# REGRAGUIahmed/DGViT-Depth-Goal-Guided-Vision-Transformer-

Hardware: AMD Instinct MI355X
Metric: depth frames/sec through DGViT fwd+bwd, batch 512x84x84 (higher is better)
Workload: dtype f32

## Files before the change

### dgvit-depth-goal-guided-vision-transformer-_amd/csrc/gemm.hip

```cpp
#include <algorithm>

#include "common.h"
#include "gemm_tile.h"

namespace {

__device__ __forceinline__ void stamp(const GemmParams& p, int slot, int tid) {
#ifdef DGVIT_DIAG
  if (p.stamps && tid == 0 && (int)blockIdx.x < p.stamp_capacity) {
    long long* s = p.stamps + (long long)blockIdx.x * 16;
    s[slot] = __builtin_readcyclecounter();
    if (slot == 0) {
      s[4] = wall_clock64();
      s[5] = (long long)__builtin_amdgcn_s_getreg((31 << 11) | 4) | ((long long)__builtin_amdgcn_s_getreg((31 << 11) | 20) << 32);
    }
    if (slot == 3) s[6] = wall_clock64();
  }
#endif
}
#ifdef DGVIT_DIAG
#define DIAG_BIT(p, b) ((p).diag & (b))
#define DIAG_STAMPS(p) ((p).stamps != nullptr)
#else
#define DIAG_BIT(p, b) 0
#define DIAG_STAMPS(p) false
#endif

__device__ __forceinline__ long long unpatch_off(const GemmParams& p, int m, int k) {
  const int b = m / p.g_P, pi = m - b * p.g_P, py = pi / p.g_gw, px = pi - py * p.g_gw;
  const int i = k / p.g_pw, j = k - i * p.g_pw;
  return (long long)b * p.g_hw + (long long)(py * p.g_ph + i) * p.g_wi + px * p.g_pw + j;
}

template <class T, int LAYOUT, int VEC, int EPI, bool GATHER = false>
__global__ void __launch_bounds__(T::NT, T::MINB) gemm_f32_kernel(const GemmParams p) {
  constexpr int BM = T::BM, BN = T::BN, BK = T::BK, NT = T::NT;
  constexpr bool AKC = LAYOUT != GEMM_TN;
  constexpr bool BKC = LAYOUT == GEMM_NT;
  constexpr bool TWO_OUT = EPI == EPI_GELU2 || EPI == EPI_GELU2D;
  constexpr bool ACT_GRAD = EPI == EPI_DGELU || EPI == EPI_DMUL;
  constexpr bool NT_STORES = TWO_OUT || ACT_GRAD;
  constexpr int WM = BM / T::WVM, WN = BN / T::WVN, TM = WM / 32, TN = WN / 32;
  static_assert(WM % 32 == 0 && WN % 32 == 0 && BM <= NT, "bad wave layout");
  constexpr int A_TILE = AKC ? BM * (BK + 4) : BK * (BM + 4);
  constexpr int B_TILE = BKC ? BN * (BK + 4) : BK * (BN + 4);
  constexpr int STAGE = A_TILE + B_TILE;
  using FA = Fetch<BM, BK, AKC, VEC, NT, GATHER>;
  using FB = Fetch<BN, BK, BKC, VEC, NT>;

  extern __shared__ __attribute__((aligned(16))) float smem[];

  const int tid = threadIdx.x, lane = tid & 63, wave = tid >> 6;
  const int li = lane & 31, h = lane >> 5;
  const int wm = wave / T::WVN, wn = wave % T::WVN;

  const int tiles_n = (p.N + BN - 1) / BN, tiles_m = (p.M + BM - 1) / BM;
  int tile, zs = 0, nz = 1;
  int zslice = blockIdx.z;
  if (EPI == EPI_SPLITK && p.zsplit > 1) {
    const int ntile = tiles_m * tiles_n, w = xcd_remap(blockIdx.x, ntile * p.zsplit);
    zslice = w / ntile;
    tile = w - zslice * ntile;
  } else if (EPI != EPI_SPLITK && p.nsplit > 1 && (int)blockIdx.x >= p.split_from) {
    const int r = (int)blockIdx.x - p.split_from;
    tile = p.split_from + r / p.nsplit;
    zs = r % p.nsplit;
    nz = p.nsplit;
  } else {
    tile = xcd_remap(blockIdx.x, EPI != EPI_SPLITK && p.nsplit > 1 ? p.split_from : tiles_m * tiles_n);
  }
  const int m0 = (tile / tiles_n) * BM, n0 = (tile % tiles_n) * BN;
  const int kbeg = nz > 1 ? zs * p.kchunk_split : zslice * p.kchunk;
  const int kend = min(p.K, kbeg + (nz > 1 ? p.kchunk_split : p.kchunk));
  const int nk = kend > kbeg ? (kend - kbeg + BK - 1) / BK : 0;

  f32x16 acc[TM][TN];
#pragma unroll
  for (int i = 0; i < TM; ++i)
#pragma unroll
    for (int j = 0; j < TN; ++j)
#pragma unroll
      for (int r = 0; r < 16; ++r) acc[i][j][r] = 0.f;

  float bsum = 0.f;
  const bool do_colsum = EPI == EPI_SPLITK && p.colsum && n0 == 0 && tid < BM;

  float4 ra[FA::NV], rb[FB::NV];
  const int klim = kend - kbeg;
  stamp(p, 0, tid);

  constexpr bool ELEMWISE = BM == 64 && BN == 64 && BK == 32;
  constexpr bool LN_OK = EPI == EPI_STORE && BN == 64 && VEC == 4 && !GATHER && LAYOUT != GEMM_TN;
  const bool evec = !ELEMWISE || p.evec;
  constexpr int CS = BN + 4;
  constexpr int NCHUNK = (BM * CS <= 2 * STAGE) ? 1 : T::WVM;
  constexpr int CROWS = BM / NCHUNK;
  static_assert(CROWS * CS <= 2 * STAGE && (NCHUNK == 1 || CROWS == WM), "epilogue C image does not fit the staging LDS");
  constexpr int C4 = BN / 4, RPP = NT / C4;
  const int cc = (tid % C4) * 4, rr0 = tid / C4;
  const int n = n0 + cc;
  constexpr bool DIRECT_OK = LAYOUT != GEMM_TN && VEC == 4 && !GATHER && EPI != EPI_SPLITK && EPI != EPI_UNPATCH && (BKC || TN <= 2);
  const bool direct = DIRECT_OK && nz == 1 && evec && p.c_rgrp == 0 && p.res_mod == 0 && (!TWO_OUT || p.ldc2 == p.ldc) && !DIAG_BIT(p, 8) &&
                      !(LN_OK && p.ln_y);
  int dcol[TN];
  float dbias[TN];
#pragma unroll
  for (int j = 0; j < TN; ++j) {
    dcol[j] = wn * WN + (BKC ? j * 32 + li : li * TN + j);
    dbias[j] = 0.f;
  }
  float bias4[4] = {0.f, 0.f, 0.f, 0.f};
  if ((EPI == EPI_STORE || TWO_OUT || EPI == EPI_RELU || EPI == EPI_GELU) && p.bias) {
    if (direct) {
#pragma unroll
      for (int j = 0; j < TN; ++j) dbias[j] = p.bias[min(n0 + dcol[j], p.N - 1)];
    } else {
#pragma unroll
      for (int e = 0; e < 4; ++e)
        if (n + e < p.N) bias4[e] = p.bias[n + e];
    }
  }

  auto load_frags = [&](float (&fa)[TM][4], float (&fb)[TN][4], const float* la, const float* lb, int g) {
    if constexpr (AKC) {
#pragma unroll
      for (int i = 0; i < TM; ++i) frag<BM, BK, true>(fa[i], la, wm * WM + i * 32 + li, g, h);
    } else {
      frag_mc<BM, TM>(fa, la, wm * WM, li, g, h);
    }
    if constexpr (BKC) {
#pragma unroll
      for (int j = 0; j < TN; ++j) frag<BN, BK, true>(fb[j], lb, wn * WN + j * 32 + li, g, h);
    } else {
      frag_mc<BN, TN>(fb, lb, wn * WN, li, g, h);
    }
  };
  auto do_mfma = [&](const float (&fa)[TM][4], const float (&fb)[TN][4]) {
#pragma unroll
    for (int s4 = 0; s4 < 4; ++s4)
#pragma unroll
      for (int i = 0; i < TM; ++i)
#pragma unroll
        for (int j = 0; j < TN; ++j)
          acc[i][j] = __builtin_amdgcn_mfma_f32_32x32x2f32(fa[i][s4], fb[j][s4], acc[i][j], 0, 0, 0);
  };
  auto mma_group = [&](const float* la, const float* lb, int g) {
    float fa[TM][4], fb[TN][4];
    load_frags(fa, fb, la, lb, g);
    do_mfma(fa, fb);
  };

  if (VEC == 4) {
    typename FA::Plan pa;
    typename FB::Plan pb;
    if constexpr (GATHER) FA::plan_gather(pa, p, m0, kbeg, tid);
    else FA::plan(pa, p.A, p.lda, m0, p.M, kbeg, p.K, tid);
    FB::plan(pb, p.B, p.ldb, n0, p.N, kbeg, p.K, tid);
    {
      float4 ra0[FA::NV], rb0[FB::NV];
      FA::run4(ra0, pa, 0, klim);
      FB::run4(rb0, pb, 0, klim);
      FA::run4(ra, pa, 1, klim);
      FB::run4(rb, pb, 1, klim);
      FA::stash(ra0, smem, tid);
      FB::stash(rb0, smem + A_TILE, tid);
    }
    __syncthreads();
    stamp(p, 1, tid);
    if (DIAG_BIT(p, 1)) __builtin_amdgcn_s_setprio(2);
    for (int kt = 0; kt < nk; ++kt) {
      const float* la = smem + (kt & 1) * STAGE;
      const float* lb = la + A_TILE;
      float* wa = smem + ((kt + 1) & 1) * STAGE;
      float fa[2][TM][4], fb[2][TN][4];
      load_frags(fa[0], fb[0], la, lb, 0);
      FA::stash(ra, wa, tid);
      FB::stash(rb, wa + A_TILE, tid);
      FA::run4(ra, pa, kt + 2, klim);
      FB::run4(rb, pb, kt + 2, klim);
#pragma unroll
      for (int g = 0; g < BK / 8; ++g) {
        if (g + 1 < BK / 8) load_frags(fa[(g + 1) & 1], fb[(g + 1) & 1], la, lb, g + 1);
        do_mfma(fa[g & 1], fb[g & 1]);
      }
      sched_pattern<4 * TM * TN, FA::NV + FB::NV, (AKC ? TM : (TM == 1 ? 2 : 4)) + (BKC ? TN : (TN == 1 ? 2 : 4)), BK / 8>();
      if (EPI == EPI_SPLITK && do_colsum) {
#pragma unroll 8
        for (int kk = 0; kk < BK; ++kk) bsum += la[kk * (BM + 4) + tid];
      }
      __syncthreads();
    }
    if (DIAG_BIT(p, 1)) __builtin_amdgcn_s_setprio(0);
  } else {
    FA::run(ra, p.A, p.lda, m0, p.M, kbeg, kend, tid);
    FB::run(rb, p.B, p.ldb, n0, p.N, kbeg, kend, tid);
    FA::stash(ra, smem, tid);
    FB::stash(rb, smem + A_TILE, tid);
    __syncthreads();
    for (int kt = 0; kt < nk; ++kt) {
      const float* la = smem + (kt & 1) * STAGE;
      const float* lb = la + A_TILE;
      const bool more = kt + 1 < nk;
      if (more) {
        FA::run(ra, p.A, p.lda, m0, p.M, kbeg + (kt + 1) * BK, kend, tid);
        FB::run(rb, p.B, p.ldb, n0, p.N, kbeg + (kt + 1) * BK, kend, tid);
      }
#pragma unroll
      for (int g = 0; g < BK / 8; ++g) mma_group(la, lb, g);
      if (EPI == EPI_SPLITK && do_colsum) {
#pragma unroll 8
        for (int kk = 0; kk < BK; ++kk) bsum += la[kk * (BM + 4) + tid];
      }
      if (more) {
        float* wa = smem + ((kt + 1) & 1) * STAGE;
        FA::stash(ra, wa, tid);
        FB::stash(rb, wa + A_TILE, tid);
      }
      __syncthreads();
    }
  }

  stamp(p, 2, tid);
  if (DIAG_BIT(p, 2)) {
    float sacc = 0.f;
#pragma unroll
    for (int i = 0; i < TM; ++i)
#pragma unroll
      for (int j = 0; j < TN; ++j)
#pragma unroll
        for (int r = 0; r < 16; ++r) sacc += acc[i][j][r];
    if (sacc == 1.2345678e33f) p.C[0] = sacc;
    return;
  }
  if constexpr (DIRECT_OK) {
    if (direct) {
      constexpr int CW = BKC ? 1 : TN;
      auto tile_rsrc = [&](const float* base, int ld) {
        long long bytes = ((long long)(p.M - 1 - m0) * ld + (p.N - n0)) * 4;
        if (bytes > 0x7FFFFFFFll) bytes = 0x7FFFFFFFll;
        return __builtin_amdgcn_make_buffer_rsrc(const_cast<float*>(base + (long long)m0 * ld + n0), 0, (int)bytes, 0x00020000);
      };
      auto eoff = [&](int i, int j, int r, int ld) -> unsigned {
        const unsigned rowpart = (unsigned)((wm * WM + i * 32 + (r & 3) + 8 * (r >> 2)) * ld * 4);
        return n0 + dcol[j] < p.N ? rowpart + (unsigned)((4 * h * ld + dcol[j]) * 4) : DGVIT_OOB;
      };
      constexpr bool HAS_SIDE = EPI == EPI_STORE || ACT_GRAD || EPI == EPI_DRELU;
      const bool use_side = HAS_SIDE && (EPI == EPI_STORE ? p.res != nullptr : true);
      if (HAS_SIDE && use_side) {
        const float* sb = EPI == EPI_STORE ? p.res : p.aux;
        const int sld = EPI == EPI_STORE ? p.ldr : p.ldaux;
        const __amdgpu_buffer_rsrc_t sr = tile_rsrc(sb, sld);
        float side[TM][16][TN];
#pragma unroll
        for (int i = 0; i < TM; ++i)
#pragma unroll
          for (int r = 0; r < 16; ++r) {
            if constexpr (CW == 2) {
              typedef float f32x2v __attribute__((ext_vector_type(2)));
              const f32x2v v2 = __builtin_bit_cast(f32x2v, __builtin_amdgcn_raw_buffer_load_b64(sr, eoff(i, 0, r, sld), 0, 0));
              side[i][r][0] = v2[0];
              side[i][r][1] = v2[1];
            } else {
#pragma unroll
              for (int j = 0; j < TN; ++j)
                side[i][r][j] = __builtin_bit_cast(float, __builtin_amdgcn_raw_buffer_load_b32(sr, eoff(i, j, r, sld), 0, 0));
            }
          }
#pragma unroll
        for (int i = 0; i < TM; ++i)
#pragma unroll
          for (int j = 0; j < TN; ++j)
#pragma unroll
            for (int r = 0; r < 16; ++r) {
              const float sv = side[i][r][j];
              if (EPI == EPI_STORE) acc[i][j][r] += sv;
              else if (EPI == EPI_DGELU) acc[i][j][r] *= gelu_erf_grad(sv);
              else if (EPI == EPI_DMUL) acc[i][j][r] *= sv;
              else acc[i][j][r] = sv > 0.f ? acc[i][j][r] : 0.f;
            }
      }
      auto st32 = [&](unsigned v, __amdgpu_buffer_rsrc_t rs, unsigned off) {
        if (NT_STORES || DIAG_BIT(p, 16)) __builtin_amdgcn_raw_buffer_store_b32(v, rs, off, 0, 2);
        else __builtin_amdgcn_raw_buffer_store_b32(v, rs, off, 0, 0);
      };
      auto st64 = [&](u32x2 v, __amdgpu_buffer_rsrc_t rs, unsigned off) {
        if (NT_STORES || DIAG_BIT(p, 16)) __builtin_amdgcn_raw_buffer_store_b64(v, rs, off, 0, 2);
        else __builtin_amdgcn_raw_buffer_store_b64(v, rs, off, 0, 0);
      };
      const __amdgpu_buffer_rsrc_t cr = tile_rsrc(p.C, p.ldc);
      __amdgpu_buffer_rsrc_t c2r = cr;
      if (TWO_OUT) c2r = tile_rsrc(p.C2, p.ldc2);
#pragma unroll
      for (int i = 0; i < TM; ++i)
#pragma unroll
        for (int r = 0; r < 16; ++r) {
          float v[TN];
#pragma unroll
          for (int j = 0; j < TN; ++j) {
            v[j] = acc[i][j][r];
            if (EPI == EPI_STORE || TWO_OUT) v[j] += dbias[j];
            else if (EPI == EPI_RELU) v[j] = fmaxf(v[j] + dbias[j], 0.f);
            else if (EPI == EPI_GELU) v[j] = gelu_erf(v[j] + dbias[j]);
          }
          if constexpr (CW == 1) {
#pragma unroll
            for (int j = 0; j < TN; ++j) {
              if constexpr (EPI == EPI_GELU2D) {
                float gl, gd;
                gelu_erf_both(v[j], gl, gd);
                st32(__builtin_bit_cast(unsigned, gd), cr, eoff(i, j, r, p.ldc));
                st32(__builtin_bit_cast(unsigned, gl), c2r, eoff(i, j, r, p.ldc));
              } else {
                st32(__builtin_bit_cast(unsigned, v[j]), cr, eoff(i, j, r, p.ldc));
                if (EPI == EPI_GELU2)
                  st32(__builtin_bit_cast(unsigned, gelu_erf(v[j])), c2r, eoff(i, j, r, p.ldc));
              }
            }
          } else {
            u32x2 w;
// ... 79 lines not shown
#pragma unroll
      for (int e = 0; e < 4; ++e) v[e] += bias4[e];
    } else if (TWO_OUT) {
#pragma unroll
      for (int e = 0; e < 4; ++e) {
        v[e] += bias4[e];
        if constexpr (EPI == EPI_GELU2D) gelu_erf_both(v[e], w2[e], v[e]);
        else w2[e] = gelu_erf(v[e]);
      }
    } else if (EPI == EPI_RELU) {
#pragma unroll
      for (int e = 0; e < 4; ++e) v[e] = fmaxf(v[e] + bias4[e], 0.f);
    } else if (EPI == EPI_GELU) {
#pragma unroll
      for (int e = 0; e < 4; ++e) v[e] = gelu_erf(v[e] + bias4[e]);
    } else if (ACT_GRAD || EPI == EPI_DRELU) {
      const float* ap = p.aux + (long long)m * p.ldaux + n;
      float a4[4] = {0.f, 0.f, 0.f, 0.f};
      if (evec) {
        const float4 q = *reinterpret_cast<const float4*>(ap);
        a4[0] = q.x; a4[1] = q.y; a4[2] = q.z; a4[3] = q.w;
      } else {
#pragma unroll
        for (int e = 0; e < 4; ++e)
          if (n + e < p.N) a4[e] = ap[e];
      }
#pragma unroll
      for (int e = 0; e < 4; ++e) v[e] = EPI == EPI_DGELU ? v[e] * gelu_erf_grad(a4[e]) : (EPI == EPI_DMUL ? v[e] * a4[e] : (a4[e] > 0.f ? v[e] : 0.f));
    }
    if (evec) {
      *reinterpret_cast<float4*>(cptr) = make_float4(v[0], v[1], v[2], v[3]);
      if (TWO_OUT) *reinterpret_cast<float4*>(p.C2 + (long long)m * p.ldc2 + n) = make_float4(w2[0], w2[1], w2[2], w2[3]);
      if (LN_OK && p.ln_y) ln_piece(m, v);
    } else {
#pragma unroll
      for (int e = 0; e < 4; ++e)
        if (n + e < p.N) {
          cptr[e] = v[e];
          if (TWO_OUT) p.C2[(long long)m * p.ldc2 + n + e] = w2[e];
        }
    }
  };
  float* slab = nullptr;
  if (EPI != EPI_SPLITK && nz > 1) slab = p.slabs + ((long long)(tile - p.split_from) * nz + zs) * (BM * BN);
  constexpr int NP = CROWS / RPP;
  static_assert(CROWS % RPP == 0, "epilogue row pieces");
  constexpr bool HAS_SIDE = EPI == EPI_STORE || ACT_GRAD || EPI == EPI_DRELU;
  constexpr bool SIDE_ALL = NCHUNK == 1 && NP <= 4;
  const bool fast = evec && !slab;
  const bool nvalid = n < p.N;
  const int nc = nvalid ? n : 0;
  const bool use_side = HAS_SIDE && (EPI == EPI_STORE ? p.res != nullptr : true);
  float4 side[HAS_SIDE ? (SIDE_ALL ? NCHUNK * NP : NP) : 1];
#pragma unroll
  for (auto& sv : side) sv = make_float4(0.f, 0.f, 0.f, 0.f);
  auto load_side = [&](int ch, float4* dst) {
#pragma unroll
    for (int it = 0; it < NP; ++it) {
      const int m = min(m0 + ch * CROWS + rr0 + it * RPP, p.M - 1);
      const float* sp;
      if (EPI == EPI_STORE) {
        const long long rrow = p.res_mod > 0 ? (long long)(m % p.res_mod) + 1 : (long long)m;
        sp = p.res + rrow * p.ldr + nc;
      } else {
        sp = p.aux + (long long)m * p.ldaux + nc;
      }
      dst[it] = *reinterpret_cast<const float4*>(sp);
    }
  };
  if (HAS_SIDE && SIDE_ALL && fast && use_side) {
#pragma unroll
    for (int ch = 0; ch < NCHUNK; ++ch) load_side(ch, side + ch * NP);
  }
#pragma unroll
  for (int ch = 0; ch < NCHUNK; ++ch) {
    if (NCHUNK == 1 || wm == ch) {
      const int rbase = NCHUNK == 1 ? wm * WM : 0;
#pragma unroll
      for (int i = 0; i < TM; ++i)
#pragma unroll
        for (int r = 0; r < 16; ++r) {
          const int rt = (r & 3) + 8 * (r >> 2) + 4 * h;
          float* crow = smem + (rbase + (AKC ? i * 32 + rt : rt * TM + i)) * CS + wn * WN;
          if constexpr (BKC || TN == 1) {
#pragma unroll
            for (int j = 0; j < TN; ++j) crow[j * 32 + li] = acc[i][j][r];
          } else {
            typedef float cvec_t __attribute__((ext_vector_type(TN)));
            cvec_t v;
#pragma unroll
            for (int j = 0; j < TN; ++j) v[j] = acc[i][j][r];
            *reinterpret_cast<cvec_t*>(crow + li * TN) = v;
          }
        }
    }
    __syncthreads();
    stamp(p, 8 + 2 * ch, tid);
    if (slab) {
      const __amdgpu_buffer_rsrc_t srs = __builtin_amdgcn_make_buffer_rsrc(slab, 0, BM * BN * 4, 0x00020000);
      for (int rr = rr0; rr < CROWS; rr += RPP) {
        const float4 t = *reinterpret_cast<const float4*>(smem + rr * CS + cc);
        __builtin_amdgcn_raw_buffer_store_b128(__builtin_bit_cast(u32x4, t), srs, (unsigned)(((ch * CROWS + rr) * BN + cc) * 4), 0, 16);
      }
    } else if (fast) {
      if (HAS_SIDE && !SIDE_ALL && use_side) load_side(ch, side);
      float4* sd = side + (HAS_SIDE && SIDE_ALL ? ch * NP : 0);
      if (EPI == EPI_DGELU) {
#pragma unroll
        for (int it = 0; it < NP; ++it)
          sd[it] = make_float4(gelu_erf_grad(sd[it].x), gelu_erf_grad(sd[it].y), gelu_erf_grad(sd[it].z), gelu_erf_grad(sd[it].w));
      }
      constexpr bool T_FIRST = NCHUNK == 1;
      float4 t[T_FIRST ? NP : 1];
      if constexpr (T_FIRST) {
#pragma unroll
        for (int it = 0; it < NP; ++it) t[it] = *reinterpret_cast<const float4*>(smem + (rr0 + it * RPP) * CS + cc);
      }
#pragma unroll
      for (int it = 0; it < NP; ++it) {
        const int m = m0 + ch * CROWS + rr0 + it * RPP;
        if constexpr (!T_FIRST) t[0] = *reinterpret_cast<const float4*>(smem + (rr0 + it * RPP) * CS + cc);
        const float4 tv = t[T_FIRST ? it : 0];
        float v[4] = {tv.x, tv.y, tv.z, tv.w}, w2[4];
        if (EPI == EPI_STORE) {
          if (use_side) { v[0] += sd[it].x; v[1] += sd[it].y; v[2] += sd[it].z; v[3] += sd[it].w; }
#pragma unroll
          for (int e = 0; e < 4; ++e) v[e] += bias4[e];
        } else if (TWO_OUT) {
#pragma unroll
          for (int e = 0; e < 4; ++e) {
            v[e] += bias4[e];
            if constexpr (EPI == EPI_GELU2D) gelu_erf_both(v[e], w2[e], v[e]);
            else w2[e] = gelu_erf(v[e]);
          }
        } else if (EPI == EPI_RELU) {
#pragma unroll
          for (int e = 0; e < 4; ++e) v[e] = fmaxf(v[e] + bias4[e], 0.f);
        } else if (EPI == EPI_GELU) {
#pragma unroll
          for (int e = 0; e < 4; ++e) v[e] = gelu_erf(v[e] + bias4[e]);
        } else if (ACT_GRAD || EPI == EPI_DRELU) {
          const float a4[4] = {sd[it].x, sd[it].y, sd[it].z, sd[it].w};
#pragma unroll
          for (int e = 0; e < 4; ++e) v[e] = ACT_GRAD ? v[e] * a4[e] : (a4[e] > 0.f ? v[e] : 0.f);
        }
        if (EPI == EPI_UNPATCH && m < p.M && nvalid) {
          *reinterpret_cast<float4*>(Cz + unpatch_off(p, m, n)) = make_float4(v[0], v[1], v[2], v[3]);
        } else if (EPI != EPI_UNPATCH && m < p.M && nvalid) {
          long long crow = m;
          if (EPI == EPI_STORE && p.c_rgrp > 0) crow = (long long)m + m / p.c_rgrp + 1;
          int ncol = n;
          if (DIAG_BIT(p, 4)) {
            crow = m - m0;
            ncol = cc;
          }
          *reinterpret_cast<float4*>(Cz + crow * p.ldc + ncol) = make_float4(v[0], v[1], v[2], v[3]);
          if (TWO_OUT) *reinterpret_cast<float4*>(p.C2 + crow * p.ldc2 + ncol) = make_float4(w2[0], w2[1], w2[2], w2[3]);
          if (LN_OK && p.ln_y) ln_piece(m, v);
        }
      }
    } else if (ELEMWISE && n < p.N) {
      for (int it = 0; it < CROWS / RPP; ++it) {
        const int rr = rr0 + it * RPP;
        const int m = m0 + ch * CROWS + rr;
        if (m < p.M) {
          const float4 t = *reinterpret_cast<const float4*>(smem + rr * CS + cc);
          float v[4] = {t.x, t.y, t.z, t.w};
// ... 252 lines not shown
```

### dgvit-depth-goal-guided-vision-transformer-_amd/csrc/gemm_tile.h

```cpp
#pragma once
#include "common.h"

namespace {

template <int BM_, int BN_, int BK_, int WVM_ = 2, int WVN_ = 2>
struct TileCfg {
  static constexpr int BM = BM_, BN = BN_, BK = BK_, WVM = WVM_, WVN = WVN_, NT = 64 * WVM_ * WVN_;
  static constexpr int LDS_BYTES = 2 * (BM_ + BN_) * (BK_ + 4) * 4;
  static constexpr int MINB = LDS_BYTES * 5 <= 160 * 1024 ? 5 : 2;
};

__device__ __forceinline__ int xcd_remap(int id, int n) {
  const int q = n >> 3, r = n & 7, xcd = id & 7, loc = id >> 3;
  return (xcd < r ? xcd * (q + 1) : r * (q + 1) + (xcd - r) * q) + loc;
}

typedef unsigned u32x4 __attribute__((ext_vector_type(4)));
typedef unsigned u32x2 __attribute__((ext_vector_type(2)));
#define DGVIT_OOB 0xFFFFFFF0u

template <int R, int BK, bool KC, int VEC, int NT, bool GATHER = false>
struct Fetch {
  static_assert(!GATHER || (KC && VEC == 4), "the patch gather is a k-contiguous float4 fetch");
  static_assert(R * BK / 4 % NT == 0, "tile must split evenly over the workgroup's threads");
  static constexpr int NV = R * BK / 4 / NT;
  static constexpr int PER_ROW = KC ? BK / 4 : R / 4;

  struct Plan {
    __amdgpu_buffer_rsrc_t rsrc;
    unsigned off[NV];
    int kc[NV];
    unsigned bad[NV];
    unsigned kstep;
    int g_wi, g_pw, g_inv, g_shift;
    int g_k0;
  };

  __device__ static __forceinline__ void plan_gather(Plan& pl, const GemmParams& p, int r0, int kbeg, int tid) {
    pl.g_k0 = kbeg;
    long long bytes = p.g_img_floats * 4;
    if (bytes > 0x7FFFFFFFll) bytes = 0x7FFFFFFFll;
    pl.rsrc = __builtin_amdgcn_make_buffer_rsrc(const_cast<float*>(p.g_img), 0, (int)bytes, 0x00020000);
    pl.kstep = 0;
    pl.g_wi = p.g_wi; pl.g_pw = p.g_pw; pl.g_inv = p.g_inv; pl.g_shift = p.g_shift ? p.g_shift : 16;
    const int xs = p.g_xs ? p.g_xs : p.g_pw;
#pragma unroll
    for (int i = 0; i < NV; ++i) {
      const int f = tid + i * NT;
      const int a = f / PER_ROW, c = (f % PER_ROW) * 4;
      const int m = r0 + a;
      const int b = m / p.g_P, pi = m - b * p.g_P, hy = pi / p.g_gw, wx = pi - hy * p.g_gw;
      pl.off[i] = ((unsigned)b * (unsigned)p.g_hw + (unsigned)(hy * p.g_ph) * (unsigned)p.g_wi + (unsigned)(wx * xs)) * 4u;
      pl.kc[i] = c;
      pl.bad[i] = m < p.M ? 0u : 0xFFFFFFFFu;
    }
  }

  __device__ static __forceinline__ void plan(Plan& pl, const float* base, int ld, int r0, int rmax, int kbeg, int ktotal,
                                              int tid) {
    long long first, last;
    if (KC) {
      first = (long long)r0 * ld + kbeg;
      last = (long long)(rmax - 1) * ld + ktotal;
    } else {
      first = (long long)kbeg * ld + r0;
      last = (long long)(ktotal - 1) * ld + rmax;
    }
    long long bytes = (last - first) * 4;
    if (bytes > 0x7FFFFFFFll) bytes = 0x7FFFFFFFll;
    if (bytes < 0) bytes = 0;
    pl.rsrc = __builtin_amdgcn_make_buffer_rsrc(const_cast<float*>(base + first), 0, (int)bytes, 0x00020000);
    pl.kstep = KC ? BK * 4u : (unsigned)BK * (unsigned)ld * 4u;
#pragma unroll
    for (int i = 0; i < NV; ++i) {
      const int f = tid + i * NT;
      const int a = f / PER_ROW, c = (f % PER_ROW) * 4;
      if (KC) {
        pl.off[i] = ((unsigned)a * (unsigned)ld + (unsigned)c) * 4u;
        pl.kc[i] = c;
        pl.bad[i] = 0u;
      } else {
        pl.off[i] = ((unsigned)a * (unsigned)ld + (unsigned)c) * 4u;
        pl.kc[i] = a;
        pl.bad[i] = r0 + c < rmax ? 0u : 0xFFFFFFFFu;
      }
    }
  }

  __device__ static __forceinline__ void run4(float4 (&reg)[NV], const Plan& pl, int t, int klim) {
#pragma unroll
    for (int i = 0; i < NV; ++i) {
      unsigned at;
      if constexpr (GATHER) {
        const unsigned k = (unsigned)(pl.g_k0 + t * BK + pl.kc[i]), p1 = (k * (unsigned)pl.g_inv) >> pl.g_shift, p2 = k - p1 * (unsigned)pl.g_pw;
        at = (pl.off[i] + (p1 * (unsigned)pl.g_wi + p2) * 4u) | pl.bad[i];
      } else {
        at = (pl.off[i] + (unsigned)t * pl.kstep) | pl.bad[i];
      }
      const unsigned o = t * BK + pl.kc[i] < klim ? at : DGVIT_OOB;
      reg[i] = __builtin_bit_cast(float4, __builtin_amdgcn_raw_buffer_load_b128(pl.rsrc, o, 0, 0));
    }
  }

  __device__ static __forceinline__ void run(float4 (&reg)[NV], const float* __restrict__ base, int ld, int r0,
                                             int rmax, int k0, int kend, int tid) {
#pragma unroll
    for (int i = 0; i < NV; ++i) {
      const int f = tid + i * NT;
      const int a = f / PER_ROW, c = (f % PER_ROW) * 4;
      float4 v = make_float4(0.f, 0.f, 0.f, 0.f);
      if (KC) {
        const int row = r0 + a, k = k0 + c;
        if (row < rmax) {
          const float* src = base + (long long)row * ld + k;
          if (k + 0 < kend) v.x = src[0];
          if (k + 1 < kend) v.y = src[1];
          if (k + 2 < kend) v.z = src[2];
          if (k + 3 < kend) v.w = src[3];
        }
      } else {
        const int k = k0 + a, col = r0 + c;
        if (k < kend) {
          const float* src = base + (long long)k * ld + col;
          if (col + 0 < rmax) v.x = src[0];
          if (col + 1 < rmax) v.y = src[1];
          if (col + 2 < rmax) v.z = src[2];
          if (col + 3 < rmax) v.w = src[3];
        }
      }
      reg[i] = v;
    }
  }

  __device__ static __forceinline__ void stash(const float4 (&reg)[NV], float* lds, int tid) {
    constexpr int STRIDE = KC ? BK + 4 : R + 4;
#pragma unroll
    for (int i = 0; i < NV; ++i) {
      const int f = tid + i * NT;
      const int a = f / PER_ROW, c = (f % PER_ROW) * 4;
      *reinterpret_cast<float4*>(lds + a * STRIDE + c) = reg[i];
    }
  }
};

template <int R, int BK, bool KC>
__device__ __forceinline__ void frag(float (&out)[4], const float* lds, int row, int g, int h) {
  if (KC) {
    const float4 v = *reinterpret_cast<const float4*>(lds + row * (BK + 4) + 8 * g + 4 * h);
    out[0] = v.x; out[1] = v.y; out[2] = v.z; out[3] = v.w;
  } else {
    const float* p = lds + (8 * g + 4 * h) * (R + 4) + row;
#pragma unroll
    for (int s = 0; s < 4; ++s) out[s] = p[s * (R + 4)];
  }
}

template <int R, int NTILE>
__device__ __forceinline__ void frag_mc(float (&out)[NTILE][4], const float* lds, int base, int li, int g, int h) {
  typedef float vec_t __attribute__((ext_vector_type(NTILE == 1 ? 1 : NTILE == 2 ? 2 : 4)));
  static_assert(NTILE == 1 || NTILE == 2 || NTILE == 4, "frag_mc: tiles per wave");
  const float* p = lds + (8 * g + 4 * h) * (R + 4) + base + NTILE * li;
#pragma unroll
  for (int s = 0; s < 4; ++s) {
    if constexpr (NTILE == 1) {
      out[0][s] = p[s * (R + 4)];
    } else {
      typedef __attribute__((address_space(3))) const volatile vec_t lds_vec_t;
      const vec_t v = *(lds_vec_t*)(p + s * (R + 4));
#pragma unroll
      for (int t = 0; t < NTILE; ++t) out[t][s] = v[t];
    }
  }
}

#define SGB(mask, n) __builtin_amdgcn_sched_group_barrier(mask, n, 0)
constexpr int cdiv_c(int a, int b) { return (a + b - 1) / b; }
template <int m, int H, int NI, int MASK>
__device__ __forceinline__ void spread() {
  if constexpr (m < H) {
    SGB(0x8, 1);
    constexpr int c = cdiv_c((m + 1) * NI, H) - cdiv_c(m * NI, H);
    if constexpr (c > 0) SGB(MASK, c);
    spread<m + 1, H, NI, MASK>();
  }
}
template <int MF, int NW, int RPG, int NG>
__device__ __forceinline__ void sched_pattern() {
  static_assert(MF >= 2 && MF % 2 == 0, "sched_pattern: MFMAs per k-group");
  SGB(0x100, RPG);
  spread<0, MF / 2, NW, 0x200>();
  if constexpr (NG > 1) SGB(0x100, RPG);
  spread<0, MF / 2, NW, 0x20>();
  if constexpr (NG > 1) { if constexpr (NG > 2) SGB(0x100, RPG); SGB(0x8, MF); }
  if constexpr (NG > 2) { if constexpr (NG > 3) SGB(0x100, RPG); SGB(0x8, MF); }
  if constexpr (NG > 3) { if constexpr (NG > 4) SGB(0x100, RPG); SGB(0x8, MF); }
// ... 9 lines not shown
```

### dgvit-depth-goal-guided-vision-transformer-_amd/csrc/last_block.hip

```cpp
#include <math.h>

#include <algorithm>

#include "kernels.h"

#define DGVIT_LOG2E 1.4426950408889634f

namespace {

constexpr int GP_WAVES = 4;
constexpr int GP_J = 4;
constexpr int HP_FRAMES = 16;
constexpr int HP_CHUNK = 256;
constexpr int WG_ROWS = 8;

__device__ __forceinline__ float fma4(const float4 a, const float4 b, float acc) {
  acc = fmaf(a.x, b.x, acc);
  acc = fmaf(a.y, b.y, acc);
  acc = fmaf(a.z, b.z, acc);
  return fmaf(a.w, b.w, acc);
}
__device__ __forceinline__ void axpy4(float a, const float4 x, float4& acc) {
  acc.x = fmaf(a, x.x, acc.x);
  acc.y = fmaf(a, x.y, acc.y);
  acc.z = fmaf(a, x.z, acc.z);
  acc.w = fmaf(a, x.w, acc.w);
}

__device__ __forceinline__ void fma4v(const float4 a, const float4 b, float4& acc) {
  acc.x = fmaf(a.x, b.x, acc.x);
  acc.y = fmaf(a.y, b.y, acc.y);
  acc.z = fmaf(a.z, b.z, acc.z);
  acc.w = fmaf(a.w, b.w, acc.w);
}
__device__ __forceinline__ float4 add4(const float4 a, const float4 b) { return make_float4(a.x + b.x, a.y + b.y, a.z + b.z, a.w + b.w); }
__device__ __forceinline__ float hsum4(const float4 a) { return (a.x + a.y) + (a.z + a.w); }

template <int J>
__device__ __forceinline__ void pool_rows(const float* __restrict__ w, const float4* __restrict__ xs4, int N, int D4, int lane, float4 (&out)[J]) {
  float4 acc[4][J];
#pragma unroll
  for (int k = 0; k < 4; ++k)
#pragma unroll
    for (int j = 0; j < J; ++j) acc[k][j] = make_float4(0.f, 0.f, 0.f, 0.f);
  int t = 0;
  for (; t + 3 < N; t += 4) {
    const float4 wv = *reinterpret_cast<const float4*>(w + t);
    const float wk[4] = {wv.x, wv.y, wv.z, wv.w};
#pragma unroll
    for (int k = 0; k < 4; ++k)
#pragma unroll
      for (int j = 0; j < J; ++j) {
        const int c = lane + 64 * j;
        if (c < D4) axpy4(wk[k], xs4[(t + k) * D4 + c], acc[k][j]);
      }
  }
  for (; t < N; ++t) {
    const float wt = w[t];
#pragma unroll
    for (int j = 0; j < J; ++j) {
      const int c = lane + 64 * j;
      if (c < D4) axpy4(wt, xs4[t * D4 + c], acc[0][j]);
    }
  }
#pragma unroll
  for (int j = 0; j < J; ++j) out[j] = add4(add4(acc[0][j], acc[1][j]), add4(acc[2][j], acc[3][j]));
}

__device__ __forceinline__ void stage_frame(const float* __restrict__ xn, float4* __restrict__ xs4, int b, int N, int D) {
  const float4* src = reinterpret_cast<const float4*>(xn + (long long)b * N * D);
  const int n4 = N * (D >> 2);
  for (int i = threadIdx.x; i < n4; i += blockDim.x) xs4[i] = src[i];
}

template <int J>
__global__ void __launch_bounds__(64 * GP_WAVES) goal_pool_fwd_kernel(const float* __restrict__ xn, const float* __restrict__ u, long long fs_u,
                                                                      float* __restrict__ r, long long fs_r, float* __restrict__ p, int N,
                                                                      int D, int H, float qscale) {
  extern __shared__ float4 gp_smem[];
  float4* xs4 = gp_smem;
  const int b = blockIdx.x, D4 = D >> 2, NP = (N + 3) & ~3;
  float* sc = reinterpret_cast<float*>(gp_smem) + (long long)N * D + (threadIdx.x >> 6) * NP;
  stage_frame(xn, xs4, b, N, D);
  __syncthreads();
  const int lane = threadIdx.x & 63;
  for (int h = threadIdx.x >> 6; h < H; h += GP_WAVES) {
    const float4* uh = reinterpret_cast<const float4*>(u + (long long)b * fs_u + (long long)h * D);
    float4 uf[J];
#pragma unroll
    for (int j = 0; j < J; ++j) {
      const int c = lane + 64 * j;
      uf[j] = c < D4 ? uh[c] : make_float4(0.f, 0.f, 0.f, 0.f);
    }
    for (int t = 0; t < N; ++t) {
      float part = 0.f;
#pragma unroll
      for (int j = 0; j < J; ++j) {
        const int c = lane + 64 * j;
        if (c < D4) part = fma4(uf[j], xs4[t * D4 + c], part);
      }
      part = wave_sum(part);
      if (lane == 0) sc[t] = part * qscale;
    }
    __builtin_amdgcn_wave_barrier();
    float m = -INFINITY;
    for (int t = lane; t < N; t += 64) m = fmaxf(m, sc[t]);
    m = wave_max(m);
    float l = 0.f;
    for (int t = lane; t < N; t += 64) {
      const float e = __builtin_amdgcn_exp2f(sc[t] - m);
      sc[t] = e;
      l += e;
    }
    l = wave_sum(l);
    const float inv = 1.f / l;
    for (int t = lane; t < N; t += 64) {
      const float pt = sc[t] * inv;
      sc[t] = pt;
      if (p) p[((long long)b * H + h) * N + t] = pt;
    }
    __builtin_amdgcn_wave_barrier();
    float4 acc[J];
    pool_rows<J>(sc, xs4, N, D4, lane, acc);
    float4* rh = reinterpret_cast<float4*>(r + (long long)b * fs_r + (long long)h * D);
#pragma unroll
    for (int j = 0; j < J; ++j) {
      const int c = lane + 64 * j;
      if (c < D4) rh[c] = acc[j];
    }
  }
}

template <int J>
__global__ void __launch_bounds__(64 * GP_WAVES) goal_pool_bwd_kernel(const float* __restrict__ xn, const float* __restrict__ p,
                                                                      const float* __restrict__ u, long long fs_u, const float* __restrict__ dr,
                                                                      float* __restrict__ du, long long fs_d, float* __restrict__ dxn, int N,
                                                                      int D, int H, float scale) {
  extern __shared__ float4 gp_smem[];
  float4* xs4 = gp_smem;
  const int b = blockIdx.x, D4 = D >> 2, NP = (N + 3) & ~3;
  float* ps = reinterpret_cast<float*>(gp_smem) + (long long)N * D;
  float* das = ps + H * NP;
  stage_frame(xn, xs4, b, N, D);
  __syncthreads();
  const int lane = threadIdx.x & 63;
  for (int h = threadIdx.x >> 6; h < H; h += GP_WAVES) {
    const float4* drh = reinterpret_cast<const float4*>(dr + (long long)b * fs_d + (long long)h * D);
    float4 df[J];
#pragma unroll
    for (int j = 0; j < J; ++j) {
      const int c = lane + 64 * j;
      df[j] = c < D4 ? drh[c] : make_float4(0.f, 0.f, 0.f, 0.f);
    }
    float* dh_ = das + h * NP;
    float* ph_ = ps + h * NP;
    for (int t = 0; t < N; ++t) {
      float part = 0.f;
#pragma unroll
      for (int j = 0; j < J; ++j) {
        const int c = lane + 64 * j;
        if (c < D4) part = fma4(df[j], xs4[t * D4 + c], part);
      }
      part = wave_sum(part);
      if (lane == 0) dh_[t] = part;
    }
    __builtin_amdgcn_wave_barrier();
    float cpart = 0.f;
    for (int t = lane; t < N; t += 64) {
      const float pt = p[((long long)b * H + h) * N + t];
      ph_[t] = pt;
      cpart = fmaf(pt, dh_[t], cpart);
    }
    const float cs = wave_sum(cpart);
    for (int t = lane; t < N; t += 64) dh_[t] = scale * (ph_[t] * (dh_[t] - cs));
    __builtin_amdgcn_wave_barrier();
    float4 acc[J];
    pool_rows<J>(dh_, xs4, N, D4, lane, acc);
    float4* duh = reinterpret_cast<float4*>(du + (long long)b * fs_d + (long long)h * D);
#pragma unroll
    for (int j = 0; j < J; ++j) {
      const int c = lane + 64 * j;
      if (c < D4) duh[c] = acc[j];
    }
  }
  __syncthreads();
  const float4* dr4 = reinterpret_cast<const float4*>(dr + (long long)b * fs_d);
  const float4* u4 = reinterpret_cast<const float4*>(u + (long long)b * fs_u);
  float4* out4 = reinterpret_cast<float4*>(dxn + (long long)b * N * D);
  const int items = ((N + 3) >> 2) * D4;
  for (int it = threadIdx.x; it < items; it += blockDim.x) {
    const int t0 = (it / D4) * 4, c = it % D4;
    float4 acc[4];
#pragma unroll
    for (int k = 0; k < 4; ++k) acc[k] = make_float4(0.f, 0.f, 0.f, 0.f);
    for (int h = 0; h < H; ++h) {
      const float4 dv = dr4[h * D4 + c], uv = u4[h * D4 + c];
      const float4 pv = *reinterpret_cast<const float4*>(ps + h * NP + t0);
      const float4 av = *reinterpret_cast<const float4*>(das + h * NP + t0);
      axpy4(pv.x, dv, acc[0]); axpy4(av.x, uv, acc[0]);
      axpy4(pv.y, dv, acc[1]); axpy4(av.y, uv, acc[1]);
      axpy4(pv.z, dv, acc[2]); axpy4(av.z, uv, acc[2]);
      axpy4(pv.w, dv, acc[3]); axpy4(av.w, uv, acc[3]);
    }
#pragma unroll
    for (int k = 0; k < 4; ++k)
      if (t0 + k < N) out4[(t0 + k) * D4 + c] = acc[k];
  }
}

template <int DH>
__global__ void __launch_bounds__(256) head_proj_kernel(const float* __restrict__ in, long long ld_in, const float* __restrict__ W,
                                                        float* __restrict__ out, long long fs_out, int B, int D) {
  __shared__ float4 in_s[HP_FRAMES][DH / 4];
  const int b0 = blockIdx.x * HP_FRAMES, h = blockIdx.y;
  for (int i = threadIdx.x; i < HP_FRAMES * (DH / 4); i += 256) {
    const int f = i / (DH / 4), k4 = i % (DH / 4);
    in_s[f][k4] = b0 + f < B ? *reinterpret_cast<const float4*>(in + (long long)(b0 + f) * ld_in + h * DH + 4 * k4) : make_float4(0.f, 0.f, 0.f, 0.f);
  }
  __syncthreads();
  for (int d = threadIdx.x; d < D; d += 256) {
    float4 acc[HP_FRAMES];
#pragma unroll
    for (int f = 0; f < HP_FRAMES; ++f) acc[f] = make_float4(0.f, 0.f, 0.f, 0.f);
    const float* wp = W + (long long)h * DH * D + d;
#pragma unroll 2
    for (int k4 = 0; k4 < DH / 4; ++k4) {
      const float4 w = make_float4(wp[(long long)(4 * k4) * D], wp[(long long)(4 * k4 + 1) * D], wp[(long long)(4 * k4 + 2) * D],
                                   wp[(long long)(4 * k4 + 3) * D]);
#pragma unroll
      for (int f = 0; f < HP_FRAMES; ++f) fma4v(in_s[f][k4], w, acc[f]);
    }
#pragma unroll
    for (int f = 0; f < HP_FRAMES; ++f)
      if (b0 + f < B) out[(long long)(b0 + f) * fs_out + (long long)h * D + d] = hsum4(acc[f]);
  }
}

template <int DH>
__global__ void __launch_bounds__(256) head_proj_t_kernel(const float* __restrict__ in, long long fs_in, const float* __restrict__ W,
                                                          float* __restrict__ out, long long ld_out, int B, int D) {
  constexpr int FPT = HP_FRAMES * DH / 256;
  __shared__ float4 in_s[HP_FRAMES][HP_CHUNK / 4];
  const int b0 = blockIdx.x * HP_FRAMES, h = blockIdx.y;
  const int j = threadIdx.x % DH, f0 = (threadIdx.x / DH) * FPT;
  const float* wrow = W + ((long long)h * DH + j) * D;
  float4 acc[FPT][4];
#pragma unroll
  for (int i = 0; i < FPT; ++i)
#pragma unroll
    for (int k = 0; k < 4; ++k) acc[i][k] = make_float4(0.f, 0.f, 0.f, 0.f);
  for (int d0 = 0; d0 < D; d0 += HP_CHUNK) {
    const int dc4 = (D - d0 < HP_CHUNK ? D - d0 : HP_CHUNK) >> 2;
    __syncthreads();
    for (int i = threadIdx.x; i < HP_FRAMES * dc4; i += 256) {
      const int f = i / dc4, c = i % dc4;
      in_s[f][c] = b0 + f < B ? *reinterpret_cast<const float4*>(in + (long long)(b0 + f) * fs_in + (long long)h * D + d0 + 4 * c)
                              : make_float4(0.f, 0.f, 0.f, 0.f);
    }
    __syncthreads();
    int c = 0;
    for (; c + 3 < dc4; c += 4) {
#pragma unroll
      for (int k = 0; k < 4; ++k) {
        const float4 w = *reinterpret_cast<const float4*>(wrow + d0 + 4 * (c + k));
#pragma unroll
        for (int i = 0; i < FPT; ++i) fma4v(in_s[f0 + i][c + k], w, acc[i][k]);
      }
    }
    for (; c < dc4; ++c) {
      const float4 w = *reinterpret_cast<const float4*>(wrow + d0 + 4 * c);
#pragma unroll
      for (int i = 0; i < FPT; ++i) fma4v(in_s[f0 + i][c], w, acc[i][0]);
    }
  }
#pragma unroll
  for (int i = 0; i < FPT; ++i)
    if (b0 + f0 + i < B)
      out[(long long)(b0 + f0 + i) * ld_out + h * DH + j] = hsum4(add4(add4(acc[i][0], acc[i][1]), add4(acc[i][2], acc[i][3])));
}

template <int DH>
__global__ void __launch_bounds__(256) head_proj_wgrad_kernel(const float* __restrict__ q, long long ld_q, const float* __restrict__ du,
                                                              long long fs_du, const float* __restrict__ dout, long long ld_do,
                                                              const float* __restrict__ r, long long fs_r, float* __restrict__ dW, int B,
                                                              int D, int H, int vec) {
  __shared__ float4 red[3][WG_ROWS][64];
  constexpr int RT = DH / WG_ROWS;
  const int z = blockIdx.z, h = blockIdx.y, rt = blockIdx.x % RT, cb = blockIdx.x / RT;
  const float* A = z ? dout : q;
  const long long lda = z ? ld_do : ld_q;
  const float* X = z ? r : du;
  const long long fsx = z ? fs_r : fs_du;
  const int lane = threadIdx.x & 63, wave = threadIdx.x >> 6;
  const int c = cb * 64 + lane, D4 = D >> 2;
  const bool valid = c < D4;
  const int chunk = (B + 3) >> 2;
  const int bb = wave * chunk, be = bb + chunk < B ? bb + chunk : B;
  float4 acc[WG_ROWS];
#pragma unroll
  for (int i = 0; i < WG_ROWS; ++i) acc[i] = make_float4(0.f, 0.f, 0.f, 0.f);
  if (valid) {
    for (int b = bb; b < be; ++b) {
      const float4 x = *reinterpret_cast<const float4*>(X + (long long)b * fsx + (long long)h * D + 4 * c);
      const float* ap = A + (long long)b * lda + h * DH + rt * WG_ROWS;
      const float4 a0 = *reinterpret_cast<const float4*>(ap), a1 = *reinterpret_cast<const float4*>(ap + 4);
      axpy4(a0.x, x, acc[0]); axpy4(a0.y, x, acc[1]); axpy4(a0.z, x, acc[2]); axpy4(a0.w, x, acc[3]);
      axpy4(a1.x, x, acc[4]); axpy4(a1.y, x, acc[5]); axpy4(a1.z, x, acc[6]); axpy4(a1.w, x, acc[7]);
    }
  }
  if (wave > 0) {
#pragma unroll
    for (int i = 0; i < WG_ROWS; ++i) red[wave - 1][i][lane] = acc[i];
  }
  __syncthreads();
  if (wave == 0 && valid) {
    const long long I = (long long)H * DH;
    float* o = dW + (z * I + (long long)h * DH + rt * WG_ROWS) * D + 4 * c;
#pragma unroll
    for (int i = 0; i < WG_ROWS; ++i) {
      float4 s = acc[i];
#pragma unroll
      for (int w = 0; w < 3; ++w) {
        const float4 v = red[w][i][lane];
        s.x += v.x; s.y += v.y; s.z += v.z; s.w += v.w;
      }
      float* oi = o + (long long)i * D;
      if (vec) *reinterpret_cast<float4*>(oi) = s;
      else { oi[0] = s.x; oi[1] = s.y; oi[2] = s.z; oi[3] = s.w; }
    }
  }
}

template <int J>
int launch_pool_fwd(const float* xn, const float* u, long long fs_u, float* r, long long fs_r, float* p, int B, int N, int D, int H, float scale,
                    hipStream_t st) {
  auto kern = goal_pool_fwd_kernel<J>;
  TRY(allow_dynamic_lds<goal_pool_fwd_kernel<J>>((int)GOAL_POOL_LDS_MAX, "goal_pool_fwd"));
  const long long np = (N + 3) & ~3;
  const size_t lds = (size_t)((long long)N * D + GP_WAVES * np) * sizeof(float);
  {
    ProfileScope t(PROF_ATTN_FWD, 4.0 * B * H * (double)N * D, st);
    hipLaunchKernelGGL(kern, dim3(B), dim3(64 * GP_WAVES), lds, st, xn, u, fs_u, r, fs_r, p, N, D, H, scale * DGVIT_LOG2E);
  }
  DGVIT_CHECK_LAUNCH("goal_pool_fwd");
  return DGVIT_OK;
}

template <int J>
int launch_pool_bwd(const float* xn, const float* p, const float* u, long long fs_u, const float* dr, float* du, long long fs_d, float* dxn,
                    int B, int N, int D, int H, float scale, hipStream_t st) {
  auto kern = goal_pool_bwd_kernel<J>;
  TRY(allow_dynamic_lds<goal_pool_bwd_kernel<J>>((int)GOAL_POOL_LDS_MAX, "goal_pool_bwd"));
  const long long np = (N + 3) & ~3;
  const size_t lds = (size_t)((long long)N * D + 2ll * H * np) * sizeof(float);
  {
    ProfileScope t(PROF_ATTN_BWD, 8.0 * B * H * (double)N * D, st);
    hipLaunchKernelGGL(kern, dim3(B), dim3(64 * GP_WAVES), lds, st, xn, p, u, fs_u, dr, du, fs_d, dxn, N, D, H, scale);
  }
  DGVIT_CHECK_LAUNCH("goal_pool_bwd");
  return DGVIT_OK;
}

}

long long goal_pool_lds_bytes(int N, int D, int H) {
  const long long np = (N + 3) & ~3;
  const long long extra = std::max<long long>(GP_WAVES, 2ll * H) * np;
  return ((long long)N * D + extra) * (long long)sizeof(float);
}

bool goal_attention_supports(int N, int D, int H, int dh) {
  return N >= 1 && H >= 1 && D >= 4 && D % 4 == 0 && D <= 256 * GP_J && (dh == 32 || dh == 64) && goal_pool_lds_bytes(N, D, H) <= GOAL_POOL_LDS_MAX;
}

#define GOAL_CHECK_SHAPE(name)                                                                                                       \
  DGVIT_CHECK_ARG(B > 0 && goal_attention_supports(N, D, H, dh),                                                                    \
                  name ": unsupported shape B=%d N=%d H=%d dim_head=%d dim=%d (dim_head 32 or 64, dim a multiple of 4 up to 1024, "  \
                       "N * dim floats within %d KB of LDS)", B, N, H, dh, D, (int)(GOAL_POOL_LDS_MAX / 1024))

int head_proj(const float* in, long long ld_in, const float* W, float* out, long long fs_out, int B, int H, int dh, int D, hipStream_t st) {
  DGVIT_CHECK_ARG(in && W && out && al16(in) && ld_in % 4 == 0, "head_proj: bad arguments");
  const dim3 grid((B + HP_FRAMES - 1) / HP_FRAMES, H);
  {
    ProfileScope t(PROF_OTHER, 2.0 * B * H * (double)dh * D, st);
    if (dh == 64) hipLaunchKernelGGL(head_proj_kernel<64>, grid, dim3(256), 0, st, in, ld_in, W, out, fs_out, B, D);
    else hipLaunchKernelGGL(head_proj_kernel<32>, grid, dim3(256), 0, st, in, ld_in, W, out, fs_out, B, D);
  }
  DGVIT_CHECK_LAUNCH("head_proj");
  return DGVIT_OK;
}
// ... 69 lines not shown
```

Measured before the change: 41280.

## Pair B columns in GEMM fetch and batch loads in last-block attention kernels

Adds a paired-row permutation to the B operand fetch when TN==2 with k-contiguous B, so each lane owns adjacent output columns and the epilogue can use vector stores. In the last-block kernels it also batches independent global and LDS loads ahead of the FMAs: tokens are processed in groups of eight with a shared wave reduction, frame staging is unrolled, heads are blocked by four, and the weight-gradient loop takes eight frames per step with WG_ROWS halved to four. The intent is more memory-level parallelism and fewer serialized wave reductions, at the cost of extra registers and possible occupancy loss.

Measured after the change: 41570, median of 6. About the same (+0.7%).

```diff
diff --git a/dgvit-depth-goal-guided-vision-transformer-_amd/csrc/gemm.hip b/dgvit-depth-goal-guided-vision-transformer-_amd/csrc/gemm.hip
--- a/dgvit-depth-goal-guided-vision-transformer-_amd/csrc/gemm.hip
+++ b/dgvit-depth-goal-guided-vision-transformer-_amd/csrc/gemm.hip
@@ -46,7 +46,8 @@
   constexpr int B_TILE = BKC ? BN * (BK + 4) : BK * (BN + 4);
   constexpr int STAGE = A_TILE + B_TILE;
   using FA = Fetch<BM, BK, AKC, VEC, NT, GATHER>;
-  using FB = Fetch<BN, BK, BKC, VEC, NT>;
+  constexpr bool BPAIR = BKC && TN == 2, BTILED = BKC && !BPAIR;
+  using FB = Fetch<BN, BK, BKC, VEC, NT, false, BPAIR>;
 
   extern __shared__ __attribute__((aligned(16))) float smem[];
 
@@ -106,7 +107,7 @@
   float dbias[TN];
 #pragma unroll
   for (int j = 0; j < TN; ++j) {
-    dcol[j] = wn * WN + (BKC ? j * 32 + li : li * TN + j);
+    dcol[j] = wn * WN + (BTILED ? j * 32 + li : li * TN + j);
     dbias[j] = 0.f;
   }
   float bias4[4] = {0.f, 0.f, 0.f, 0.f};
@@ -234,7 +235,7 @@
   }
   if constexpr (DIRECT_OK) {
     if (direct) {
-      constexpr int CW = BKC ? 1 : TN;
+      constexpr int CW = BTILED ? 1 : TN;
       auto tile_rsrc = [&](const float* base, int ld) {
         long long bytes = ((long long)(p.M - 1 - m0) * ld + (p.N - n0)) * 4;
         if (bytes > 0x7FFFFFFFll) bytes = 0x7FFFFFFFll;
@@ -480,7 +481,7 @@
         for (int r = 0; r < 16; ++r) {
           const int rt = (r & 3) + 8 * (r >> 2) + 4 * h;
           float* crow = smem + (rbase + (AKC ? i * 32 + rt : rt * TM + i)) * CS + wn * WN;
-          if constexpr (BKC || TN == 1) {
+          if constexpr (BTILED || TN == 1) {
 #pragma unroll
             for (int j = 0; j < TN; ++j) crow[j * 32 + li] = acc[i][j][r];
           } else {
diff --git a/dgvit-depth-goal-guided-vision-transformer-_amd/csrc/gemm_tile.h b/dgvit-depth-goal-guided-vision-transformer-_amd/csrc/gemm_tile.h
--- a/dgvit-depth-goal-guided-vision-transformer-_amd/csrc/gemm_tile.h
+++ b/dgvit-depth-goal-guided-vision-transformer-_amd/csrc/gemm_tile.h
@@ -19,9 +19,11 @@
 typedef unsigned u32x2 __attribute__((ext_vector_type(2)));
 #define DGVIT_OOB 0xFFFFFFF0u
 
-template <int R, int BK, bool KC, int VEC, int NT, bool GATHER = false>
+template <int R, int BK, bool KC, int VEC, int NT, bool GATHER = false, bool PAIRED = false>
 struct Fetch {
   static_assert(!GATHER || (KC && VEC == 4), "the patch gather is a k-contiguous float4 fetch");
+  static_assert(!PAIRED || (KC && !GATHER && R % 64 == 0), "column pairs: a k-contiguous operand in 64-row wave blocks");
+  __device__ static __forceinline__ int src_row(int a) { return PAIRED ? (a & ~63) + 2 * (a & 31) + ((a >> 5) & 1) : a; }
   static_assert(R * BK / 4 % NT == 0, "tile must split evenly over the workgroup's threads");
   static constexpr int NV = R * BK / 4 / NT;
   static constexpr int PER_ROW = KC ? BK / 4 : R / 4;
@@ -76,7 +78,7 @@
       const int f = tid + i * NT;
       const int a = f / PER_ROW, c = (f % PER_ROW) * 4;
       if (KC) {
-        pl.off[i] = ((unsigned)a * (unsigned)ld + (unsigned)c) * 4u;
+        pl.off[i] = ((unsigned)src_row(a) * (unsigned)ld + (unsigned)c) * 4u;
         pl.kc[i] = c;
         pl.bad[i] = 0u;
       } else {
@@ -110,7 +112,7 @@
       const int a = f / PER_ROW, c = (f % PER_ROW) * 4;
       float4 v = make_float4(0.f, 0.f, 0.f, 0.f);
       if (KC) {
-        const int row = r0 + a, k = k0 + c;
+        const int row = r0 + src_row(a), k = k0 + c;
         if (row < rmax) {
           const float* src = base + (long long)row * ld + k;
           if (k + 0 < kend) v.x = src[0];
diff --git a/dgvit-depth-goal-guided-vision-transformer-_amd/csrc/last_block.hip b/dgvit-depth-goal-guided-vision-transformer-_amd/csrc/last_block.hip
--- a/dgvit-depth-goal-guided-vision-transformer-_amd/csrc/last_block.hip
+++ b/dgvit-depth-goal-guided-vision-transformer-_amd/csrc/last_block.hip
@@ -10,9 +10,13 @@
 
 constexpr int GP_WAVES = 4;
 constexpr int GP_J = 4;
+constexpr int GP_TB = 8;
+constexpr int GP_STAGE = 8;
+constexpr int GP_HB = 4;
 constexpr int HP_FRAMES = 16;
 constexpr int HP_CHUNK = 256;
-constexpr int WG_ROWS = 8;
+constexpr int WG_ROWS = 4;
+constexpr int WG_FRAMES = 8;
 
 __device__ __forceinline__ float fma4(const float4 a, const float4 b, float acc) {
   acc = fmaf(a.x, b.x, acc);
@@ -43,34 +47,81 @@
   for (int k = 0; k < 4; ++k)
 #pragma unroll
     for (int j = 0; j < J; ++j) acc[k][j] = make_float4(0.f, 0.f, 0.f, 0.f);
+  int cc[J];
+#pragma unroll
+  for (int j = 0; j < J; ++j) cc[j] = lane + 64 * j < D4 ? lane + 64 * j : 0;
   int t = 0;
   for (; t + 3 < N; t += 4) {
     const float4 wv = *reinterpret_cast<const float4*>(w + t);
     const float wk[4] = {wv.x, wv.y, wv.z, wv.w};
 #pragma unroll
-    for (int k = 0; k < 4; ++k)
-#pragma unroll
-      for (int j = 0; j < J; ++j) {
-        const int c = lane + 64 * j;
-        if (c < D4) axpy4(wk[k], xs4[(t + k) * D4 + c], acc[k][j]);
-      }
+    for (int j = 0; j < J; ++j) {
+      float4 x[4];
+#pragma unroll
+      for (int k = 0; k < 4; ++k) x[k] = xs4[(t + k) * D4 + cc[j]];
+#pragma unroll
+      for (int k = 0; k < 4; ++k) axpy4(wk[k], x[k], acc[k][j]);
+    }
   }
   for (; t < N; ++t) {
     const float wt = w[t];
 #pragma unroll
+    for (int j = 0; j < J; ++j) axpy4(wt, xs4[t * D4 + cc[j]], acc[0][j]);
+  }
+#pragma unroll
+  for (int j = 0; j < J; ++j) out[j] = add4(add4(acc[0][j], acc[1][j]), add4(acc[2][j], acc[3][j]));
+}
+
+template <int J>
+__device__ __forceinline__ void dot_rows(const float4 (&f)[J], const float4* __restrict__ xs4, int N, int D4, int lane, float mul,
+                                         float* __restrict__ out) {
+  for (int t0 = 0; t0 < N; t0 += GP_TB) {
+    float part[GP_TB];
+#pragma unroll
+    for (int k = 0; k < GP_TB; ++k) part[k] = 0.f;
+#pragma unroll
     for (int j = 0; j < J; ++j) {
-      const int c = lane + 64 * j;
-      if (c < D4) axpy4(wt, xs4[t * D4 + c], acc[0][j]);
-    }
-  }
-#pragma unroll
-  for (int j = 0; j < J; ++j) out[j] = add4(add4(acc[0][j], acc[1][j]), add4(acc[2][j], acc[3][j]));
+      const bool cv = lane + 64 * j < D4;
+      const int cc = cv ? lane + 64 * j : 0;
+      float4 x[GP_TB];
+#pragma unroll
+      for (int k = 0; k < GP_TB; ++k) x[k] = xs4[min(t0 + k, N - 1) * D4 + cc];
+#pragma unroll
+      for (int k = 0; k < GP_TB; ++k) {
+        const float v = fma4(f[j], x[k], part[k]);
+        part[k] = cv ? v : part[k];
+      }
+    }
+#pragma unroll
+    for (int o = 32; o > 0; o >>= 1)
+#pragma unroll
+      for (int k = 0; k < GP_TB; ++k) part[k] += __shfl_xor(part[k], o, 64);
+    if (lane == 0) {
+      if (t0 + GP_TB <= N) {
+#pragma unroll
+        for (int k = 0; k < GP_TB; k += 4)
+          *reinterpret_cast<float4*>(out + t0 + k) = make_float4(part[k] * mul, part[k + 1] * mul, part[k + 2] * mul, part[k + 3] * mul);
+      } else {
+#pragma unroll
+        for (int k = 0; k < GP_TB; ++k)
+          if (t0 + k < N) out[t0 + k] = part[k] * mul;
+      }
+    }
+  }
 }
 
 __device__ __forceinline__ void stage_frame(const float* __restrict__ xn, float4* __restrict__ xs4, int b, int N, int D) {
   const float4* src = reinterpret_cast<const float4*>(xn + (long long)b * N * D);
   const int n4 = N * (D >> 2);
-  for (int i = threadIdx.x; i < n4; i += blockDim.x) xs4[i] = src[i];
+  constexpr int NT = 64 * GP_WAVES;
+  for (int i0 = threadIdx.x; i0 < n4; i0 += GP_STAGE * NT) {
+    float4 v[GP_STAGE];
+#pragma unroll
+    for (int k = 0; k < GP_STAGE; ++k) v[k] = src[min(i0 + k * NT, n4 - 1)];
+#pragma unroll
+    for (int k = 0; k < GP_STAGE; ++k)
+      if (i0 + k * NT < n4) xs4[i0 + k * NT] = v[k];
+  }
 }
 
 template <int J>
@@ -92,16 +143,7 @@
       const int c = lane + 64 * j;
       uf[j] = c < D4 ? uh[c] : make_float4(0.f, 0.f, 0.f, 0.f);
     }
-    for (int t = 0; t < N; ++t) {
-      float part = 0.f;
-#pragma unroll
-      for (int j = 0; j < J; ++j) {
-        const int c = lane + 64 * j;
-        if (c < D4) part = fma4(uf[j], xs4[t * D4 + c], part);
-      }
-      part = wave_sum(part);
-      if (lane == 0) sc[t] = part * qscale;
-    }
+    dot_rows<J>(uf, xs4, N, D4, lane, qscale, sc);
     __builtin_amdgcn_wave_barrier();
     float m = -INFINITY;
     for (int t = lane; t < N; t += 64) m = fmaxf(m, sc[t]);
@@ -154,16 +196,7 @@
     }
     float* dh_ = das + h * NP;
     float* ph_ = ps + h * NP;
-    for (int t = 0; t < N; ++t) {
-      float part = 0.f;
-#pragma unroll
-      for (int j = 0; j < J; ++j) {
-        const int c = lane + 64 * j;
-        if (c < D4) part = fma4(df[j], xs4[t * D4 + c], part);
-      }
-      part = wave_sum(part);
-      if (lane == 0) dh_[t] = part;
-    }
+    dot_rows<J>(df, xs4, N, D4, lane, 1.f, dh_);
     __builtin_amdgcn_wave_barrier();
     float cpart = 0.f;
     for (int t = lane; t < N; t += 64) {
@@ -193,14 +226,26 @@
     float4 acc[4];
 #pragma unroll
     for (int k = 0; k < 4; ++k) acc[k] = make_float4(0.f, 0.f, 0.f, 0.f);
-    for (int h = 0; h < H; ++h) {
-      const float4 dv = dr4[h * D4 + c], uv = u4[h * D4 + c];
-      const float4 pv = *reinterpret_cast<const float4*>(ps + h * NP + t0);
-      const float4 av = *reinterpret_cast<const float4*>(das + h * NP + t0);
-      axpy4(pv.x, dv, acc[0]); axpy4(av.x, uv, acc[0]);
-      axpy4(pv.y, dv, acc[1]); axpy4(av.y, uv, acc[1]);
-      axpy4(pv.z, dv, acc[2]); axpy4(av.z, uv, acc[2]);
-      axpy4(pv.w, dv, acc[3]); axpy4(av.w, uv, acc[3]);
+    for (int h0 = 0; h0 < H; h0 += GP_HB) {
+      float4 dv[GP_HB], uv[GP_HB];
+#pragma unroll
+      for (int k = 0; k < GP_HB; ++k) {
+        const int h = min(h0 + k, H - 1);
+        dv[k] = dr4[h * D4 + c];
+        uv[k] = u4[h * D4 + c];
+      }
+#pragma unroll
+      for (int k = 0; k < GP_HB; ++k) {
+        const int h = h0 + k;
+        if (h < H) {
+          const float4 pv = *reinterpret_cast<const float4*>(ps + h * NP + t0);
+          const float4 av = *reinterpret_cast<const float4*>(das + h * NP + t0);
+          axpy4(pv.x, dv[k], acc[0]); axpy4(av.x, uv[k], acc[0]);
+          axpy4(pv.y, dv[k], acc[1]); axpy4(av.y, uv[k], acc[1]);
+          axpy4(pv.z, dv[k], acc[2]); axpy4(av.z, uv[k], acc[2]);
+          axpy4(pv.w, dv[k], acc[3]); axpy4(av.w, uv[k], acc[3]);
+        }
+      }
     }
 #pragma unroll
     for (int k = 0; k < 4; ++k)
@@ -300,12 +345,25 @@
 #pragma unroll
   for (int i = 0; i < WG_ROWS; ++i) acc[i] = make_float4(0.f, 0.f, 0.f, 0.f);
   if (valid) {
-    for (int b = bb; b < be; ++b) {
-      const float4 x = *reinterpret_cast<const float4*>(X + (long long)b * fsx + (long long)h * D + 4 * c);
-      const float* ap = A + (long long)b * lda + h * DH + rt * WG_ROWS;
-      const float4 a0 = *reinterpret_cast<const float4*>(ap), a1 = *reinterpret_cast<const float4*>(ap + 4);
-      axpy4(a0.x, x, acc[0]); axpy4(a0.y, x, acc[1]); axpy4(a0.z, x, acc[2]); axpy4(a0.w, x, acc[3]);
-      axpy4(a1.x, x, acc[4]); axpy4(a1.y, x, acc[5]); axpy4(a1.z, x, acc[6]); axpy4(a1.w, x, acc[7]);
+    const float* xp = X + (long long)h * D + 4 * c;
+    const float* ap = A + h * DH + rt * WG_ROWS;
+    int b = bb;
+    for (; b + WG_FRAMES <= be; b += WG_FRAMES) {
+      float4 x[WG_FRAMES], a[WG_FRAMES];
+#pragma unroll
+      for (int f = 0; f < WG_FRAMES; ++f) {
+        x[f] = *reinterpret_cast<const float4*>(xp + (long long)(b + f) * fsx);
+        a[f] = *reinterpret_cast<const float4*>(ap + (long long)(b + f) * lda);
+      }
+#pragma unroll
+      for (int f = 0; f < WG_FRAMES; ++f) {
+        axpy4(a[f].x, x[f], acc[0]); axpy4(a[f].y, x[f], acc[1]); axpy4(a[f].z, x[f], acc[2]); axpy4(a[f].w, x[f], acc[3]);
+      }
+    }
+    for (; b < be; ++b) {
+      const float4 x = *reinterpret_cast<const float4*>(xp + (long long)b * fsx);
+      const float4 a = *reinterpret_cast<const float4*>(ap + (long long)b * lda);
+      axpy4(a.x, x, acc[0]); axpy4(a.y, x, acc[1]); axpy4(a.z, x, acc[2]); axpy4(a.w, x, acc[3]);
     }
   }
   if (wave > 0) {
```
